# simonrw/rust-tensorflow-serving2

Measured on AMD Instinct MI355X. Metric: Predict RPCs/sec + p50 latency, ResNet-50 batch=1/32 at 1/2/4/8 MI355X, higher is better.
Workload: dtype bf16

## Files before the change

rust_tensorflow_serving2_amd/graph/fused.py:

```python
from __future__ import annotations

import os
from typing import Dict, List, Optional, Sequence, Set, Tuple

import numpy as np
import torch
import torch.nn.functional as F

from ..utils import tensors as T
from . import ops as O
from .ir import Graph, Node
from .placement import to_device, zeros

BF16 = torch.bfloat16
IGEMM_ONLY_ACTS = ("relu6", "hard_swish", "swish")
_CLOSING_ACTS = {"Relu": "relu", "Relu6": "relu6", "_HardSwish": "hard_swish", "_Swish": "swish"}


def _const(g: Graph, ref) -> Optional[torch.Tensor]:
    n = g.nodes.get(ref[0])
    if n is None or n.op != "Const" or n.value is None:
        return None
    v = n.value[ref[1]] if ref[1] < len(n.value) else None
    return v if isinstance(v, torch.Tensor) else None
# ... 78 lines not shown
        del g.nodes[n.name]
    last.op = op
    last.inputs = list(inputs)
    last.ctrl = ctrl
    last.attrs = attrs
    last.value = None
    return last


def _pad_k(w_nk: torch.Tensor, mult: int = 64) -> torch.Tensor:
    n, k = w_nk.shape
    kp = -(-k // mult) * mult
    if kp != k:
        w_nk = torch.cat([w_nk, torch.zeros(n, kp - k, dtype=w_nk.dtype, device=w_nk.device)], dim=1)
    return w_nk


def _to_bf16(x: torch.Tensor) -> torch.Tensor:
    if x.dtype == BF16:
        return x
    if x.dtype == torch.float32 and x.is_cuda and x.is_contiguous():
        from ..ops import hip
        return hip().cast_bf16(x)
    return x.to(BF16).contiguous()


class _Window:

    def _set_window(self, kh: int, kw: int, strides, padding: str, pads):
        self.kh, self.kw = kh, kw
        self.sh, self.sw = strides
        self.padding = padding
        self.pads = pads

    def pads_for(self, h, w):
        if self.padding == "SAME":
            return O.tf_same_pads(h, self.kh, self.sh) + O.tf_same_pads(w, self.kw, self.sw)
        if self.padding == "EXPLICIT":
            return tuple(self.pads)
        return (0, 0, 0, 0)

    def out_hw(self, h, w, pads, kh=None, kw=None):
        pt, pb, pl, pr = pads
        kh, kw = self.kh if kh is None else kh, self.kw if kw is None else kw
        return (h + pt + pb - kh) // self.sh + 1, (w + pl + pr - kw) // self.sw + 1


def _grouped_conv_torch(x: torch.Tensor, w_hwio: torch.Tensor, bias: torch.Tensor, strides, pads, groups: int):
    pt, pb, pl, pr = pads
    xc = x.permute(0, 3, 1, 2)
    xc = F.pad(xc, [pl, pr, pt, pb]) if (pt or pb or pl or pr) else xc
    y = F.conv2d(xc, w_hwio.to(x.dtype).permute(3, 2, 0, 1), stride=tuple(strides), groups=groups)
    return y.permute(0, 2, 3, 1) + bias.to(x.dtype)


class FusedConv(_Window):

    def __init__(self, w_hwio: torch.Tensor, bias: torch.Tensor, strides, padding: str, pads, act: str,
                 device: torch.device, use_hip: bool, name: str):
        kh, kw, self.cin, self.cout = w_hwio.shape
        self._set_window(kh, kw, strides, padding, pads)
        self.act = act
        self.use_hip = use_hip
        self.name = name
        self.device = device
        self.c4 = use_hip and self.cin <= 4 and self.kw <= 8
        self.khp = self.kh + (self.kh % 2) if self.c4 else self.kh
        if use_hip:
            if self.c4:
                w4 = torch.zeros(self.khp, 8, 4, self.cout, device=w_hwio.device)
                w4[:self.kh, :self.kw, :self.cin, :] = w_hwio.float()
                w_nk = w4.permute(3, 0, 1, 2).reshape(self.cout, self.khp * 32)
            else:
                k = self.kh * self.kw * self.cin
                w_nk = w_hwio.permute(3, 0, 1, 2).reshape(self.cout, k)
            self.w = to_device(_pad_k(w_nk).to(BF16), device)
            self.b = to_device(bias.float(), device)
        else:
            self.w_ref = to_device(w_hwio.float(), device)
            self.b_ref = to_device(bias.float(), device)

    post = None
    post_mode = None

    def set_post(self, scale: torch.Tensor, shift: torch.Tensor, act: str, mode: str):
        dev = self.device if self.use_hip else (self.w_ref.device if hasattr(self, "w_ref") else "cpu")
        self.post = (to_device(scale.float(), dev), to_device(shift.float(), dev), act)
        self.post_mode = mode

    def post_ok(self) -> bool:
        return not self.use_hip or (not self.c4 and self.cin % 64 == 0 and self.cout % 8 == 0 and
                                    self.act not in IGEMM_ONLY_ACTS)

    def _hwio(self) -> torch.Tensor:
        if not self.use_hip:
            return self.w_ref
        if self.c4:
            w = self.w[:, :self.khp * 32].reshape(self.cout, self.khp, 8, 4)[:, :self.kh, :self.kw, :self.cin]
        else:
            w = self.w[:, :self.kh * self.kw * self.cin].reshape(self.cout, self.kh, self.kw, self.cin)
        return w.float().permute(1, 2, 3, 0)

    def _torch(self, x, res, pads):
        w = self._hwio().to(x.device)
        b = (self.b if self.use_hip else self.b_ref).to(x.device)
        y = _grouped_conv_torch(x.float(), w, b, (self.sh, self.sw), pads, x.shape[3] // self.cin)
        if res is not None:
            y = y + res.float()
        outs = _with_post(self, _ref_act(y, self.act).contiguous())
        return [o.to(BF16) for o in outs] if self.use_hip else outs

    def __call__(self, ctx, node, ins):
        x = O.to_torch(ins[0])
        res = O.to_torch(ins[1]) if len(ins) > 1 else None
        pt, pb, pl, pr = self.pads_for(x.shape[1], x.shape[2])
        if not self.use_hip or x.shape[3] != self.cin:
            return self._torch(x, res, (pt, pb, pl, pr))
        from ..ops import ACT, hip, tuned_config
        if self.c4:
            ho, wo = self.out_hw(x.shape[1], x.shape[2], (pt, pb, pl, pr))
            hp, wp = (ho - 1) * self.sh + self.khp, (wo - 1) * self.sw + 8
            x = hip().ingest_c4_padded(x.float().contiguous(), hp, wp, pt, pl)
            pt = pb = pl = pr = 0
        elif self.cin % 8 != 0:
            x = x.float().contiguous()
        else:
            x = _to_bf16(x).contiguous()
        H = hip()
        n, h, w, _ = x.shape
        kh, kw = (self.khp, 8) if self.c4 else (self.kh, self.kw)
        ho, wo = self.out_hw(h, w, (pt, pb, pl, pr), kh, kw)
        if res is not None:
            res = _residual_for(res, (n, ho, wo, self.cout))
            if res is None:
                return _add_residual_unfused(self, ctx, node, ins[0], O.to_torch(ins[1]))
            res = _to_bf16(res).contiguous()
        M = n * ho * wo
        args = (x, self.w, self.b, res, kh, kw, self.sh, self.sw, pt, pb, pl, pr, ACT[self.act])
        out = torch.empty((n, ho, wo, self.cout), device=x.device, dtype=BF16)
        K = kh * 32 if self.c4 else kh * kw * self.cin
        dma = not self.c4 and self.cin % 8 == 0
        aligned = (dma and self.cin % 64 == 0) or self.c4
        halo_shape = aligned and not self.c4 and kh == 3 and kw == 3 and self.sh == 1
        halo = halo_shape and self.sw == 1 and pt <= 2 and pl <= 2
        key = ("conv", tuple(x.shape), x.dtype, self.cout, kh, kw, self.sh, res is not None, self.act,
               self.post_mode) + ((self.sw,) if self.sw != self.sh else ()) + \
            (("nohalo",) if halo_shape and self.sw == 1 and not halo else ())
        kw_post, outs = _post_kwargs(self, out)
        run = lambda c, s: H.conv2d(*args, cfg=c, out=out, splits=s, **kw_post)
        flags = {"relu6": True} if self.act in IGEMM_ONLY_ACTS else {}
        cfg, splits = tuned_config(key, M, self.cout, run, K, dma, aligned, halo=halo,
                                   cgemm_only=self.post is not None, stem=self.c4, **flags)
        run(cfg, splits)
        return outs


class FusedDepthwiseConv(_Window):

    MAX_K = 7

    def __init__(self, w_hwc: torch.Tensor, bias: torch.Tensor, strides, padding: str, pads, act: str,
                 device: torch.device, use_hip: bool, name: str):
        kh, kw, self.c = w_hwc.shape
        self._set_window(kh, kw, strides, padding, pads)
        self.act = act
        self.use_hip = use_hip
        self.name = name
        self.device = device
        self.w = to_device(w_hwc.float().contiguous(), device)
        self.b = to_device(bias.float(), device)

    @classmethod
    def hip_ok(cls, kh: int, kw: int, c: int) -> bool:
        return c % 8 == 0 and kh <= cls.MAX_K and kw <= cls.MAX_K

    def _torch(self, x, pads):
        w = self.w.to(x.device).reshape(self.kh, self.kw, 1, self.c)
        return _grouped_conv_torch(x.float(), w, self.b.to(x.device), (self.sh, self.sw), pads, self.c)

    def __call__(self, ctx, node, ins):
        x = O.to_torch(ins[0])
        pt, pb, pl, pr = self.pads_for(x.shape[1], x.shape[2])
        n, h, w, _ = x.shape
        ho, wo = self.out_hw(h, w, (pt, pb, pl, pr))
        if not self.use_hip:
            return [_ref_act(self._torch(x, (pt, pb, pl, pr)), self.act).contiguous()]
        from ..ops import ACT, hip, tuned_choice
        H = hip()
        x = _to_bf16(x).contiguous()
        out = torch.empty((n, ho, wo, self.c), device=x.device, dtype=BF16)

        def run(strip):
            return H.dwconv2d(x, self.w, self.b, self.kh, self.kw, self.sh, self.sw, pt, pl, ho, wo, ACT[self.act],
                              out, strip)
        auto = H.dwconv_strip(n, ho, wo, self.c, self.kh, self.kw, self.sh, self.sw)
        if auto == 0:
            forms = H.dwconv_forms(n, ho, wo, self.c, self.kh, self.kw, self.sh, self.sw)
            if len(forms) == 1:
                return [run(0)]
            key = ("dwconv5x5", tuple(x.shape), self.sh, self.sw, pt, pl, ho, wo, self.act)
            pick = tuned_choice(key, {int(f): (lambda f=int(f): run(f)) for f in forms}, default=0)
            return [run(pick)]
        key = ("dwconv", tuple(x.shape), self.kh, self.kw, self.sh, self.sw, pt, pl, ho, wo, self.act)
# ... 652 lines not shown

    children = ("conv", "pool")

    def __init__(self, conv: FusedConv, pool: MaxPool):
        self.conv, self.pool = conv, pool
        self.use_hip = conv.use_hip and conv.c4

    def accepts_bf16_input(self, pos: int) -> bool:
        return pos == 0 and self.use_hip

    def __call__(self, ctx, node, ins):
        x = O.to_torch(ins[0])
        conv, pool = self.conv, self.pool
        if not (self.use_hip and x.is_cuda and x.dim() == 4):
            return pool(ctx, node, conv(ctx, node, [x]))
        from ..ops import ACT, hip
        pt, pb, pl, pr = conv.pads_for(x.shape[1], x.shape[2])
        hc, wc = conv.out_hw(x.shape[1], x.shape[2], (pt, pb, pl, pr))
        ppt, ppb, ppl, ppr = pool.pads_for(hc, wc)
        kw = {}
        if pool.post is not None:
            sc, sh, act = pool.post
            kw = dict(post_scale=sc, post_shift=sh, post_act=ACT[act])
        x = x.contiguous() if x.dtype == torch.bfloat16 else x.float().contiguous()
        return [hip().stem_pool(x, conv.w, conv.b, pt, pb, pl, pr, ACT[conv.act],
                                ppt, ppb, ppl, ppr, **kw)]


O.OPS["_StemPool"] = _impl_op

CHAIN_SHAPES_ALL = {(64, 256, 64), (64, 256, 128), (128, 512, 128), (128, 512, 256)}
CHAIN_SHAPES_STAGE1 = {(64, 256, 64), (64, 256, 128)}
CHAIN_SHAPES_DUAL = {(128, 256, 64)}
CHAIN_SHAPES_DEFAULT = CHAIN_SHAPES_ALL


class ChainConv:

    children = ("a", "b")

    def __init__(self, a, b: FusedConv):
        self.a, self.b = a, b
        self.dual = isinstance(a, FusedDualConv)
        self.use_hip = a.use_hip and b.use_hip
        self.name = a.name
        if self.dual:
            from types import SimpleNamespace
            self.subs = [(a, SimpleNamespace(op="_FusedDualConv")), (b, SimpleNamespace(op="_FusedConv2D"))]

    def __call__(self, ctx, node, ins):
        x = O.to_torch(ins[0])
        a, b = self.a, self.b

        def split():
            y1 = a(ctx, node, ins)[0]
            return [y1, b(ctx, node, [y1])[0]]
        if self.dual:
            return self._call_dual(x, O.to_torch(ins[1]), split)
        res = O.to_torch(ins[1]) if len(ins) > 1 else None
        if not (self.use_hip and x.is_cuda and x.dim() == 4 and x.shape[-1] == a.cin) or \
                (res is not None and tuple(res.shape) != tuple(x.shape[:3]) + (a.cout,)):
            return split()
        from ..ops import ACT, hip, tuned_choice
        xb = _to_bf16(x).contiguous()
        rb = None if res is None else _to_bf16(res).contiguous()

        def chained():
            return list(hip().conv_chain(xb, a.w, a.b, rb, ACT[a.act], b.w, b.b, ACT[b.act]))
        key = ("chain", tuple(x.shape), a.cout, b.cout, res is not None, a.act, b.act)
        dflt = 1 if (a.cin, a.cout, b.cout) in CHAIN_SHAPES_STAGE1 else 0
        pick = tuned_choice(key, {1: chained, 0: split}, default=dflt)
        return chained() if pick == 1 else split()

    def _call_dual(self, h, x, split):
        a, b = self.a, self.b
        if not (self.use_hip and h.is_cuda and h.dim() == 4 and x.dim() == 4 and h.shape[:3] == x.shape[:3] and
                h.shape[-1] == a.c1 and x.shape[-1] == a.c2):
            return split()
        from ..ops import ACT, hip, tuned_choice
        hb, xb = _to_bf16(h).contiguous(), _to_bf16(x).contiguous()

        def chained():
            return list(hip().conv_chain(hb, a.w, a.b, None, ACT[a.act], b.w, b.b, ACT[b.act], x2=xb))
        key = ("chain", tuple(h.shape), a.cout, b.cout, ("dual", a.c2), a.act, b.act)
        dflt = 1 if (a.c1 + a.c2, a.cout, b.cout) in CHAIN_SHAPES_DUAL else 0
        pick = tuned_choice(key, {1: chained, 0: split}, default=dflt)
        return chained() if pick == 1 else split()


O.OPS["_ChainConv"] = _impl_op
O.OPS["_FusedMatMulLN"] = _impl_op

_PASSTHROUGH = ("Identity", "Squeeze", "Reshape")


def fuse_classifier_head(g, order, fed, fetch_refs, device, opts):
    c = _Ctx(g, order, fed, fetch_refs, device, opts)

    def single(node) -> bool:
        return node.name not in c.fetch_nodes and len(c.cons.get(node.name, [])) == 1

    def walk(ref, chain):
        n = g.nodes.get(ref[0])
        while n is not None and n.op in _PASSTHROUGH and ref[1] == 0 and single(n) and n.inputs:
            chain.append(n)
            ref = n.inputs[0]
            n = g.nodes.get(ref[0])
        return ref, n
# ... 975 lines not shown
```

rust_tensorflow_serving2_amd/kernels/bindings.cpp:

```cpp
#include <cstdlib>
#include <cmath>
#include <algorithm>
#include <torch/extension.h>
#include <ATen/hip/impl/HIPGuardImplMasqueradingAsCUDA.h>
#include <ATen/hip/impl/HIPStreamMasqueradingAsCUDA.h>

#include "common.h"
#include "launch.h"
#include "cgemm.h"

namespace {

using torch::Tensor;

hipStream_t cur_stream(const Tensor& t) {
  return c10::hip::getCurrentHIPStreamMasqueradingAsCUDA(t.device().index()).stream();
}

void check(hipError_t e, const char* what) {
  TORCH_CHECK(e == hipSuccess, what, ": ", hipGetErrorString(e));
}

const tfsk::TileConfig* config_of(int64_t cfg) {
  return cfg >= 0 && cfg < tfsk::kTileIdEnd ? tfsk::tile_config(int(cfg)) : nullptr;
// ... 611 lines not shown
  check(tfsk::stem_pool_launch(xin.data_ptr(), xb16, bf16p(w), int(w.size(1)), bias.data_ptr<float>(), bf16p_mut(y), N,
                               H, W, C, cout, int(PT), int(PL), Hc, Wc, int(PPT), int(PPL), Hp, Wp, int(act), sc, sh,
                               int(post_act), cur_stream(x)), "stem_pool");
  return y;
}

std::vector<Tensor> conv_chain(const Tensor& x, const Tensor& w1, const Tensor& b1,
                               const c10::optional<Tensor>& residual, int64_t act1, const Tensor& w2,
                               const Tensor& b2, int64_t act2, const c10::optional<Tensor>& x2) {
  need(x, at::kBFloat16, "x");
  need(w1, at::kBFloat16, "w1");
  need(w2, at::kBFloat16, "w2");
  need(b1, at::kFloat, "b1");
  need(b2, at::kFloat, "b2");
  TORCH_CHECK(x.dim() == 4, "conv_chain: x must be NHWC");
  const bool dual = x2.has_value();
  const int Ka = x.size(3);
  const uint16_t* x2p = nullptr;
  if (dual) {
    need(*x2, at::kBFloat16, "x2");
    TORCH_CHECK(x2->dim() == 4 && x2->size(0) == x.size(0) && x2->size(1) == x.size(1) && x2->size(2) == x.size(2),
                "conv_chain: x2 must have x's n, h, w");
    TORCH_CHECK(Ka % 64 == 0 && x2->size(3) % 64 == 0 && x2->size(3) > 0,
                "conv_chain: both sources' channels must be multiples of 64");
    TORCH_CHECK(x2->device() == x.device(), "conv_chain: tensors on different devices");
    x2p = bf16p(*x2);
  }
  const int K1 = Ka + (dual ? int(x2->size(3)) : 0), N1 = w1.size(0), N2 = w2.size(0);
  TORCH_CHECK(w1.dim() == 2 && w2.dim() == 2 && w1.size(1) >= K1 && w2.size(1) >= N1 && w1.size(1) % 8 == 0 &&
                  w2.size(1) % 8 == 0, "conv_chain: w1 [N1][>= K1], w2 [N2][>= N1]");
  TORCH_CHECK(tfsk::conv_chain_supported(K1, N1, N2, dual), "conv_chain: unsupported shape K1=", K1, " N1=", N1,
              " N2=", N2, dual ? " (dual)" : "");
  TORCH_CHECK(b1.numel() == N1 && b2.numel() == N2, "conv_chain: bias sizes");
  TORCH_CHECK(w1.device() == x.device() && w2.device() == x.device() && b1.device() == x.device() &&
                  b2.device() == x.device(), "conv_chain: tensors on different devices");
  const uint16_t* rp = nullptr;
  if (residual.has_value()) {
    need(*residual, at::kBFloat16, "residual");
    TORCH_CHECK(residual->dim() == 4 && residual->size(0) == x.size(0) && residual->size(1) == x.size(1) &&
                    residual->size(2) == x.size(2) && residual->size(3) == N1, "conv_chain: residual [n][h][w][N1]");
    rp = bf16p(*residual);
  }
  c10::hip::HIPGuardMasqueradingAsCUDA guard(x.device());
  const int M = x.size(0) * x.size(1) * x.size(2);
  Tensor y1 = torch::empty({x.size(0), x.size(1), x.size(2), N1}, x.options());
  Tensor y2 = torch::empty({x.size(0), x.size(1), x.size(2), N2}, x.options());
  check(tfsk::conv_chain_launch(bf16p(x), bf16p(w1), int(w1.size(1)), b1.data_ptr<float>(), rp, bf16p_mut(y1),
                                bf16p(w2), int(w2.size(1)), b2.data_ptr<float>(), bf16p_mut(y2), M, K1, N1, N2,
                                int(act1), int(act2), cur_stream(x), x2p, Ka),
        "conv_chain");
  return {y1, y2};
}

Tensor global_avgpool(const Tensor& x, const c10::optional<Tensor>& out) {
  need(x, at::kBFloat16, "x");
  TORCH_CHECK(x.dim() == 4 && x.size(3) % 8 == 0, "global_avgpool: NHWC with C % 8 == 0");
  c10::hip::HIPGuardMasqueradingAsCUDA guard(x.device());
  const int N = x.size(0), HW = x.size(1) * x.size(2), C = x.size(3);
  Tensor y = out.has_value() ? *out : torch::empty({N, C}, x.options());
  need(y, at::kBFloat16, "out");
  check(tfsk::global_avgpool_nhwc_launch(bf16p(x), bf16p_mut(y), N, HW, C, cur_stream(x)), "gap");
  return y;
}

std::vector<Tensor> softmax_argmax(const Tensor& logits, bool want_probs, bool want_classes,
                                   const c10::optional<Tensor>& probs_out,
                                   const c10::optional<Tensor>& classes_out) {
  TORCH_CHECK(logits.is_cuda() && logits.dim() >= 1 && logits.stride(-1) == 1 &&
                  (logits.is_contiguous() || logits.dim() == 2),
              "logits must be a GPU tensor with unit column stride (contiguous, or 2-D with a row stride)");
  const bool bf = logits.scalar_type() == at::kBFloat16;
  TORCH_CHECK(bf || logits.scalar_type() == at::kFloat, "logits must be f32 or bf16");
  c10::hip::HIPGuardMasqueradingAsCUDA guard(logits.device());
  const int cols = logits.size(-1);
  const int rows = logits.numel() / cols;
  const long ld = logits.dim() == 2 ? long(logits.stride(0)) : long(cols);
  TORCH_CHECK(ld >= cols, "logits row stride");
  Tensor probs, classes;
  if (want_probs) {
    probs = probs_out.has_value() ? *probs_out : torch::empty(logits.sizes(), logits.options().dtype(at::kFloat));
    need(probs, at::kFloat, "probs");
  }
  if (want_classes) {
    auto sz = logits.sizes().vec();
    sz.pop_back();
    classes = classes_out.has_value() ? *classes_out : torch::empty(sz, logits.options().dtype(at::kLong));
    need(classes, at::kLong, "classes");
  }
  check(tfsk::softmax_argmax_launch(logits.data_ptr(), bf, want_probs ? probs.data_ptr<float>() : nullptr,
                                    want_classes ? classes.data_ptr<int64_t>() : nullptr, rows, cols, ld,
                                    cur_stream(logits)), "softmax_argmax");
  return {probs, classes};
}

std::tuple<Tensor, Tensor, bool> classifier_head_impl(const Tensor& x, const Tensor& w, const Tensor& bias, int64_t n,
                                                      int64_t probs_host, int64_t classes_host);

std::vector<Tensor> classifier_head(const Tensor& x, const Tensor& w, const Tensor& bias, int64_t n) {
  auto r = classifier_head_impl(x, w, bias, n, 0, 0);
  return {std::get<0>(r), std::get<1>(r)};
}

std::tuple<Tensor, Tensor, bool> classifier_head_impl(const Tensor& x, const Tensor& w, const Tensor& bias, int64_t n,
                                                      int64_t probs_host, int64_t classes_host) {
  need(x, at::kBFloat16, "x");
  need(w, at::kBFloat16, "w");
// ... 278 lines not shown
              "window_attention: operands must be smaller than 2 GiB");
  TORCH_CHECK(aligned16(qkv), "window_attention: qkv must be 16-byte aligned");
  TORCH_CHECK(aligned16(bias), "window_attention: bias must be 16-byte aligned");
  Tensor y = out.has_value() ? *out : torch::empty({R, heads * D}, qkv.options());
  need(y, at::kBFloat16, "out");
  TORCH_CHECK(y.numel() == R * heads * D, "window_attention: out has the wrong size");
  TORCH_CHECK(aligned16(y), "window_attention: out must be 16-byte aligned");
  TORCH_CHECK(tfsk::window_attention_supported(R, S, heads, D, nW, g.Hf, g.Wf, g.ws, g.shift),
              "window_attention: unsupported launch");
  check(tfsk::window_attention_launch(bf16p(qkv), bias.data_ptr<float>(), mp, bf16p_mut(y), R, int(S), int(heads),
                                      int(nW), float(scale), int(g.Hf), int(g.Wf), int(g.ws), int(g.shift),
                                      cur_stream(qkv)),
        "window_attention");
  return y;
}

Tensor patch_tokens(const Tensor& x, const Tensor& table, const c10::optional<Tensor>& out) {
  need(x, at::kBFloat16, "x");
  need(table, at::kFloat, "table");
  TORCH_CHECK(x.dim() == 3, "patch_tokens: x must be [B, P, C]");
  TORCH_CHECK(table.dim() == 2 && table.size(0) == x.size(1) + 1 && table.size(1) == x.size(2),
              "patch_tokens: table must be [P + 1, C]");
  const int64_t B = x.size(0), P = x.size(1), C = x.size(2);
  TORCH_CHECK(C % 8 == 0, "patch_tokens: C % 8 != 0 (C = ", C, ")");
  TORCH_CHECK(aligned16(x), "patch_tokens: x must be 16-byte aligned");
  TORCH_CHECK(aligned16(table), "patch_tokens: table must be 16-byte aligned");
  c10::hip::HIPGuardMasqueradingAsCUDA guard(x.device());
  Tensor y = out.has_value() ? *out : torch::empty({B, P + 1, C}, x.options());
  need(y, at::kBFloat16, "out");
  TORCH_CHECK(y.numel() == B * (P + 1) * C, "patch_tokens: out has the wrong size");
  TORCH_CHECK(aligned16(y), "patch_tokens: out must be 16-byte aligned");
  TORCH_CHECK(tfsk::patch_tokens_supported(B, P, C), "patch_tokens: operands must be smaller than 2 GiB");
  check(tfsk::patch_tokens_launch(bf16p(x), table.data_ptr<float>(), bf16p_mut(y), B, P, C, cur_stream(x)),
        "patch_tokens");
  return y;
}

}

PYBIND11_MODULE(TORCH_EXTENSION_NAME, m) {
  m.doc() = "gfx950 HIP kernels (MFMA implicit-GEMM conv/GEMM, attention, norms, pooling)";
  m.def("conv2d", &conv2d, "NHWC implicit-GEMM conv (+bias +residual +act)", py::arg("x"), py::arg("w"),
        py::arg("bias"), py::arg("residual"), py::arg("kh"), py::arg("kw"), py::arg("sh"), py::arg("sw"),
        py::arg("pt"), py::arg("pb"), py::arg("pl"), py::arg("pr"), py::arg("act") = 0, py::arg("cfg") = 0,
        py::arg("out") = py::none(), py::arg("out_f32") = false, py::arg("splits") = 1,
        py::arg("post_scale") = py::none(), py::arg("post_shift") = py::none(), py::arg("post_act") = 0,
        py::arg("out2") = py::none(), py::arg("post_only") = false);
  m.def("conv_chain", &conv_chain, "expand 1x1 (+residual, act) -> next reduce 1x1 (+act) in one kernel",
        py::arg("x"), py::arg("w1"), py::arg("b1"), py::arg("residual"), py::arg("act1"), py::arg("w2"),
        py::arg("b2"), py::arg("act2"), py::arg("x2") = py::none());
  m.def("conv_chain_supported", [](int64_t k1, int64_t n1, int64_t n2, bool dual) {
    return tfsk::conv_chain_supported(int(k1), int(n1), int(n2), dual);
  }, py::arg("k1"), py::arg("n1"), py::arg("n2"), py::arg("dual") = false);
  m.def("conv2d_dual", &conv2d_dual, "act(conv1x1(h) + conv1x1_stride(x) + bias) as one K-concatenated GEMM",
        py::arg("h"), py::arg("x"), py::arg("w"), py::arg("bias"), py::arg("sh"), py::arg("sw"), py::arg("act") = 0,
        py::arg("cfg") = 36, py::arg("out") = py::none(), py::arg("splits") = 1,
        py::arg("post_scale") = py::none(), py::arg("post_shift") = py::none(), py::arg("post_act") = 0,
        py::arg("out2") = py::none(), py::arg("post_only") = false);
  m.def("linear_lnx", &linear_lnx,
        "GEMM whose A / residual rows are LayerNorm inputs (statistics as partials), optionally "
        "returning its own rows' partials: {y, partials}",
        py::arg("x"), py::arg("w"), py::arg("bias"), py::arg("residual"), py::arg("act"), py::arg("cfg"),
        py::arg("out_f32") = false, py::arg("out") = py::none(), py::arg("a_st") = py::none(),
        py::arg("a_colsum") = py::none(), py::arg("a_eps") = 1e-12, py::arg("r_st") = py::none(),
        py::arg("r_gamma") = py::none(), py::arg("r_beta") = py::none(), py::arg("r_eps") = 1e-12,
        py::arg("stats") = false);
  m.def("linear", &linear,"x @ w^T (+bias +residual +act)", py::arg("x"), py::arg("w"), py::arg("bias"),
        py::arg("residual") = py::none(), py::arg("act") = 0, py::arg("cfg") = 0, py::arg("out_f32") = false,
        py::arg("alpha") = 1.0, py::arg("out") = py::none(), py::arg("splits") = 1);
  m.def("stem_pool", &stem_pool, py::arg("x"), py::arg("w"), py::arg("bias"), py::arg("pt"), py::arg("pb"),
        py::arg("pl"), py::arg("pr"), py::arg("act"), py::arg("ppt"), py::arg("ppb"), py::arg("ppl"), py::arg("ppr"),
        py::arg("post_scale") = py::none(), py::arg("post_shift") = py::none(), py::arg("post_act") = 0);
  m.def("maxpool", &maxpool, py::arg("x"), py::arg("kh"), py::arg("kw"), py::arg("sh"), py::arg("sw"),
        py::arg("pt"), py::arg("pb"), py::arg("pl"), py::arg("pr"), py::arg("out") = py::none(),
        py::arg("post_scale") = py::none(), py::arg("post_shift") = py::none(), py::arg("post_act") = 0);
  m.def("dwconv2d", &dwconv2d, "depthwise conv: act(conv(x, w [KH*KW][C] f32) + bias), NHWC bf16", py::arg("x"),
        py::arg("w"), py::arg("bias"), py::arg("kh"), py::arg("kw"), py::arg("sh"), py::arg("sw"), py::arg("pt"),
        py::arg("pl"), py::arg("ho"), py::arg("wo"), py::arg("act") = 0, py::arg("out") = py::none(),
        py::arg("strip") = 0);
  m.def("dwconv_strip", [](int64_t n, int64_t ho, int64_t wo, int64_t c, int64_t kh, int64_t kw, int64_t sh,
                           int64_t sw) {
    return tfsk::dwconv_strip(int(n), int(ho), int(wo), int(c), int(kh), int(kw), int(sh), int(sw));
  }, "output rows per thread dwconv2d picks by itself (0: the generic kernel, which has no strips)");
  m.def("dwconv_forms", [](int64_t n, int64_t ho, int64_t wo, int64_t c, int64_t kh, int64_t kw, int64_t sh,
                           int64_t sw) {
    int forms[tfsk::kDwMaxForms];
    const int k = tfsk::dwconv_forms(int(n), int(ho), int(wo), int(c), int(kh), int(kw), int(sh), int(sw), forms);
    return std::vector<int64_t>(forms, forms + k);
  }, "the strip values dwconv2d takes for the shape: [0], [0, 2, 8] (3 x 3 strips) or [0, 2, 4] (5 x 5 strips)");
  m.def("dwconv_ln", &dwconv_ln, "depthwise 7x7 conv + bias + LayerNorm over C in one launch, NHWC bf16",
        py::arg("x"), py::arg("w"), py::arg("bias"), py::arg("gamma"), py::arg("beta"), py::arg("eps"), py::arg("pt"),
        py::arg("pl"), py::arg("ho"), py::arg("wo"), py::arg("out") = py::none(), py::arg("kh") = 7,
        py::arg("kw") = 7, py::arg("sh") = 1, py::arg("sw") = 1);
  m.def("dwconv_ln_supported", [](int64_t n, int64_t ho, int64_t wo, int64_t c, int64_t kh, int64_t kw, int64_t sh,
                                  int64_t sw) {
    return tfsk::dwconv_ln_supported(n, ho, wo, c, int(kh), int(kw), int(sh), int(sw));
  }, "whether dwconv_ln takes the shape: 7 x 7, stride 1, C % 8 == 0, 8 <= C <= dwconv_ln_max_c");
  m.def("dwconv_ln_grid", [](int64_t n, int64_t ho, int64_t wo, int64_t c) {
    return int64_t(tfsk::dwconv_ln_grid(n, ho, wo, c));
  }, "workgroups of the dwconv_ln launch for the shape (0: nothing to launch or unsupported)");
  m.attr("dwconv_ln_max_c") = int64_t(tfsk::kDwLnMaxC);
  m.def("gconv2d", &gconv2d, "grouped 3x3 conv on MFMA: act(conv(x, w packed bf16) + bias), NHWC bf16", py::arg("x"),
        py::arg("w"), py::arg("bias"), py::arg("cg"), py::arg("sh"), py::arg("pt"), py::arg("pl"), py::arg("ho"),
        py::arg("wo"), py::arg("act") = 0, py::arg("out") = py::none(), py::arg("cg_out") = -1, py::arg("sw") = -1,
        py::arg("kh") = 3, py::arg("kw") = 3);
  m.def("gconv_supported", [](int64_t c, int64_t cg_in, int64_t cg_out, int64_t kh, int64_t kw, int64_t sh,
// ... 138 lines not shown
```

rust_tensorflow_serving2_amd/kernels/launch.h:

```cpp
#pragma once
#include <hip/hip_runtime.h>
#include <stdint.h>

#include "tile_configs.h"

namespace tfsk {

struct IGemmArgs {
  const void* a;
  const uint16_t* b;
  int M, N, K;
  int lda, ldb;
  int H, W, C, KH, KW, SH, SW, PT, PL, Ho, Wo;
  const float* bias;
  const uint16_t* residual;
  int ldr;
  int act;
  void* out;
  int ldc;
  int out_f32;
  float alpha;
  int splits;
  int kt_per_split;
  float* ws;
// ... 2 lines not shown
  const void* a2;
  int64_t a2_bytes;
  int K1;
  int TH, TW, TI;
  void* out2;
  const float* scale2;
  const float* shift2;
  int act2;
  int* counters;
  long long* trace;
  int trace_cap;
  int epi_f32;
  float* st_out;
  const float* a_st;
  const float* a_colsum;
  int a_parts;
  float a_eps;
  const float* r_st;
  const float* r_gamma;
  const float* r_beta;
  int r_parts;
  float r_eps;
};

int* splitk_counters(int n, hipStream_t s);
void splitk_counters_prepare(hipStream_t s);
void splitk_counters_set_owner(int64_t owner);
void splitk_counters_add_stream(int64_t owner, hipStream_t s);
int64_t splitk_counters_release(int64_t owner);
int64_t splitk_counters_reclaim();
int64_t splitk_counters_pending();
int64_t splitk_counters_captured_in_use();

enum AMode : int { kADense = 0, kAIm2col = 1, kAStemF32 = 2, kAStem7x7x3 = 3, kAC4 = 4, kADual = 5 };

hipError_t ingest_c4_launch(const float* x, uint16_t* y, int64_t pixels, int C, hipStream_t stream);

hipError_t ingest_c4_pad_launch(const float* x, uint16_t* y, int N, int H, int W, int C, int Hp, int Wp, int pt,
                               int pl, hipStream_t stream);

hipError_t splitk_reduce_launch(const IGemmArgs& args, hipStream_t stream);

hipError_t igemm_launch(const IGemmArgs& args, int a_mode, int cfg, hipStream_t stream);

hipError_t stem_pool_launch(const void* x, bool x_bf16, const uint16_t* w, int ldw, const float* bias, uint16_t* y,
                            int N, int H, int W, int C, int cout, int pt, int pl, int Hc, int Wc, int ppt, int ppl,
                            int Hp, int Wp, int act, const float* pscale, const float* pshift, int pact,
                            hipStream_t s);
bool conv_chain_supported(int K1, int N1, int N2, bool dual = false);
hipError_t conv_chain_launch(const uint16_t* x, const uint16_t* w1, int ldw1, const float* b1, const uint16_t* res,
                             uint16_t* y1, const uint16_t* w2, int ldw2, const float* b2, uint16_t* y2, int M, int K1,
                             int N1, int N2, int act1, int act2, hipStream_t s, const uint16_t* x2 = nullptr,
                             int K1a = 0);
hipError_t maxpool_nhwc_launch(const uint16_t* x, uint16_t* y, int N, int H, int W, int C,
                               int KH, int KW, int SH, int SW, int PT, int PL, int Ho, int Wo,
                               hipStream_t stream, const float* scale = nullptr, const float* shift = nullptr,
                               int act = 0);
constexpr int kDwStripShort = 2, kDwStripTall = 8;
constexpr int kDwStrip5Short = 2, kDwStrip5Tall = 4;
constexpr int kDwMaxForms = 3;
int dwconv_strip(int N, int Ho, int Wo, int C, int KH, int KW, int SH, int SW, int strip = 0);
int dwconv_forms(int N, int Ho, int Wo, int C, int KH, int KW, int SH, int SW, int* forms);
hipError_t dwconv_nhwc_launch(const uint16_t* x, const float* w, const float* bias, uint16_t* y, int N, int H, int W,
                              int C, int KH, int KW, int SH, int SW, int PT, int PL, int Ho, int Wo, int act,
                              int strip, hipStream_t stream);
constexpr int kDwLnMaxC = 1024;
constexpr int kDwLnRowsTall = 4, kDwLnRowsShort = 2;
bool dwconv_ln_supported(long N, long Ho, long Wo, long C, int KH, int KW, int SH, int SW);
long dwconv_ln_grid(long N, long Ho, long Wo, long C);
hipError_t dwconv_ln_launch(const uint16_t* x, const float* w, const float* bias, const float* gamma,
                            const float* beta, uint16_t* y, int N, int H, int W, int C, int KH, int KW, int SH, int SW,
                            int PT, int PL, int Ho, int Wo, float eps, hipStream_t stream);
constexpr int kGconvSlab = 32;
constexpr int gconv_ksteps(int cg) { return (9 * cg + 31) / 32; }
bool gconv_supported(int C, int CGin, int CGout, int KH, int KW, int SH, int SW);
long gconv_packed_elems(int C, int CG);
hipError_t gconv_nhwc_launch(const uint16_t* x, const uint16_t* w, const float* bias, uint16_t* y, int N, int H, int W,
                             int C, int CGin, int CGout, int KH, int KW, int SH, int SW, int PT, int PL, int Ho,
                             int Wo, int act, hipStream_t stream);
constexpr int kSeMaxC = 2048, kSeMaxCr = 512;
bool se_gate_supported(long B, long HW, long C, long Cr);
hipError_t se_gate_launch(const uint16_t* x, const float* w1, const float* b1, const float* w2, const float* b2,
                          float* gate, int B, int HW, int C, int Cr, int act1, int gate_act, hipStream_t stream);
hipError_t se_scale_launch(const uint16_t* x, const float* gate, uint16_t* y, int B, int HW, int C,
                           hipStream_t stream);
hipError_t global_avgpool_nhwc_launch(const uint16_t* x, uint16_t* y, int N, int HW, int C,
                                      hipStream_t stream);
hipError_t classifier_head_launch(const uint16_t* x, const uint16_t* w, const float* bias, float* ws,
                                  float* probs, int64_t* classes, int M, int HW, int K, int Np, int N,
                                  hipStream_t s, int* counter = nullptr, float* probs_h = nullptr,
                                  int64_t* classes_h = nullptr);
size_t classifier_head_ws_floats(int M, int K, int Np);
bool classifier_head_one_launch(int M, int HW, int K, int Np, int N);
hipError_t dense_softmax_launch(const float* x, int ldx, const uint16_t* w, int ldw, const float* bias,
                                float* probs, int rows, int N, int K, hipStream_t s);
hipError_t key_mask_adder_launch(const void* m, int is_int, float one, float scale, float* out, int64_t n,
                                 hipStream_t s);
hipError_t softmax_argmax_launch(const void* logits, int in_bf16, float* probs, int64_t* classes,
                                 int rows, int cols, long ld, hipStream_t stream);
hipError_t cast_f32_bf16_launch(const float* x, uint16_t* y, int64_t n, hipStream_t stream);
hipError_t cast_bf16_f32_launch(const uint16_t* x, float* y, int64_t n, hipStream_t stream);
int epi_f32_env();
hipError_t h2d_rows_launch(const void* host, void* dev, int64_t bytes, hipStream_t stream);

hipError_t layernorm_launch(const uint16_t* x, const uint16_t* r, const float* gamma, const float* beta,
                            uint16_t* y, int rows, int cols, float eps, hipStream_t stream);
// ... 46 lines not shown
```

Measured before the change: 57100.

## Add row-panel 1x1 conv kernel keeping A in registers for wide expansions

```diff
diff --git a/rust_tensorflow_serving2_amd/graph/fused.py b/rust_tensorflow_serving2_amd/graph/fused.py
--- a/rust_tensorflow_serving2_amd/graph/fused.py
+++ b/rust_tensorflow_serving2_amd/graph/fused.py
@@ -154,6 +154,18 @@
     xc = F.pad(xc, [pl, pr, pt, pb]) if (pt or pb or pl or pr) else xc
     y = F.conv2d(xc, w_hwio.to(x.dtype).permute(3, 2, 0, 1), stride=tuple(strides), groups=groups)
     return y.permute(0, 2, 3, 1) + bias.to(x.dtype)
+
+
+_PANEL = os.environ.get("TFSERVE_PANEL", "1") != "0"
+
+
+def panel_eligible(kh, kw, sh, sw, pads, cin, cout, act, post=None, c4=False) -> bool:
+    return (kh == 1 and kw == 1 and sh == 1 and sw == 1 and not any(pads) and cin in (128, 256, 512) and
+            cout % 64 == 0 and cout >= 2 * cin and act in ("none", "relu") and post is None and not c4)
+
+
+def panel_key(x_shape, cout, has_res, act):
+    return ("panel", tuple(x_shape), cout, bool(has_res), act)
 
 
 class FusedConv(_Window):
@@ -212,12 +224,32 @@
         outs = _with_post(self, _ref_act(y, self.act).contiguous())
         return [o.to(BF16) for o in outs] if self.use_hip else outs
 
-    def __call__(self, ctx, node, ins):
+    def panel_choice(self, ctx, node, ins) -> Optional[int]:
+        x = O.to_torch(ins[0])
+        res = O.to_torch(ins[1]) if len(ins) > 1 else None
+        if not (_PANEL and self.use_hip and x.is_cuda and x.dim() == 4 and x.shape[3] == self.cin):
+            return None
+        if not panel_eligible(self.kh, self.kw, self.sh, self.sw, self.pads_for(x.shape[1], x.shape[2]), self.cin,
+                              self.cout, self.act, self.post, self.c4):
+            return None
+        if res is not None and tuple(res.shape) != tuple(x.shape[:3]) + (self.cout,):
+            return None
+        from ..ops import hip, tuned_choice
+        forms = hip().conv1x1_panel_forms(x.shape[0] * x.shape[1] * x.shape[2], self.cout, self.cin)
+        if not forms:
+            return None
+        opts = {i: (lambda i=i: self(ctx, node, ins, panel_pick=i)) for i in range(len(forms) + 1)}
+        pick = tuned_choice(panel_key(x.shape, self.cout, res is not None, self.act), opts, default=0)
+        return pick if pick in opts else 0
+
+    def __call__(self, ctx, node, ins, panel_pick=None):
         x = O.to_torch(ins[0])
         res = O.to_torch(ins[1]) if len(ins) > 1 else None
         pt, pb, pl, pr = self.pads_for(x.shape[1], x.shape[2])
         if not self.use_hip or x.shape[3] != self.cin:
             return self._torch(x, res, (pt, pb, pl, pr))
+        if panel_pick is None:
+            panel_pick = self.panel_choice(ctx, node, ins)
         from ..ops import ACT, hip, tuned_config
         if self.c4:
             ho, wo = self.out_hw(x.shape[1], x.shape[2], (pt, pb, pl, pr))
@@ -251,6 +283,10 @@
         kw_post, outs = _post_kwargs(self, out)
         run = lambda c, s: H.conv2d(*args, cfg=c, out=out, splits=s, **kw_post)
         flags = {"relu6": True} if self.act in IGEMM_ONLY_ACTS else {}
+        if panel_pick:
+            bm, ns = H.conv1x1_panel_forms(M, self.cout, self.cin)[panel_pick - 1]
+            H.conv1x1_panel(x, self.w, self.b, res, ACT[self.act], bm, ns, out=out)
+            return outs
         cfg, splits = tuned_config(key, M, self.cout, run, K, dma, aligned, halo=halo,
                                    cgemm_only=self.post is not None, stem=self.c4, **flags)
         run(cfg, splits)
@@ -1009,8 +1045,10 @@
         x = O.to_torch(ins[0])
         a, b = self.a, self.b
 
+        pp = a.panel_choice(ctx, node, ins) if isinstance(a, FusedConv) else None
+
         def split():
-            y1 = a(ctx, node, ins)[0]
+            y1 = (a(ctx, node, ins) if pp is None else a(ctx, node, ins, panel_pick=pp))[0]
             return [y1, b(ctx, node, [y1])[0]]
         if self.dual:
             return self._call_dual(x, O.to_torch(ins[1]), split)
diff --git a/rust_tensorflow_serving2_amd/kernels/bindings.cpp b/rust_tensorflow_serving2_amd/kernels/bindings.cpp
--- a/rust_tensorflow_serving2_amd/kernels/bindings.cpp
+++ b/rust_tensorflow_serving2_amd/kernels/bindings.cpp
@@ -687,6 +687,40 @@
   return {y1, y2};
 }
 
+Tensor conv1x1_panel(const Tensor& x, const Tensor& w, const Tensor& bias, const c10::optional<Tensor>& residual,
+                     int64_t act, int64_t bm, int64_t nsplit, const c10::optional<Tensor>& out) {
+  need(x, at::kBFloat16, "x");
+  need(w, at::kBFloat16, "w");
+  need(bias, at::kFloat, "bias");
+  TORCH_CHECK(x.dim() == 4, "conv1x1_panel: x must be NHWC");
+  const int64_t M64 = x.size(0) * x.size(1) * x.size(2);
+  const int K = x.size(3), N = w.size(0);
+  TORCH_CHECK(w.dim() == 2 && w.size(1) >= K && w.size(1) % 8 == 0, "conv1x1_panel: w [N][>= K, a multiple of 8]");
+  TORCH_CHECK(M64 < (int64_t(1) << 31) && tfsk::conv1x1_panel_supported(int(M64), N, K, int(bm), int(nsplit)),
+              "conv1x1_panel: unsupported shape M=", M64, " N=", N, " K=", K, " bm=", bm, " nsplit=", nsplit);
+  TORCH_CHECK(act == tfsk::kActNone || act == tfsk::kActRelu, "conv1x1_panel: act must be none or relu");
+  TORCH_CHECK(bias.numel() == N, "conv1x1_panel: bias size");
+  TORCH_CHECK(w.device() == x.device() && bias.device() == x.device(), "conv1x1_panel: tensors on different devices");
+  const uint16_t* rp = nullptr;
+  if (residual.has_value()) {
+    need(*residual, at::kBFloat16, "residual");
+    TORCH_CHECK(residual->dim() == 4 && residual->size(0) == x.size(0) && residual->size(1) == x.size(1) &&
+                    residual->size(2) == x.size(2) && residual->size(3) == N && residual->device() == x.device(),
+                "conv1x1_panel: residual [n][h][w][N]");
+    rp = bf16p(*residual);
+  }
+  c10::hip::HIPGuardMasqueradingAsCUDA guard(x.device());
+  Tensor y = out.has_value() ? *out : torch::empty({x.size(0), x.size(1), x.size(2), N}, x.options());
+  need(y, at::kBFloat16, "out");
+  TORCH_CHECK(y.numel() == M64 * N && y.device() == x.device(), "conv1x1_panel: out [n][h][w][N]");
+  TORCH_CHECK(aligned16(x) && aligned16(w) && aligned16(bias) && aligned16(y) && (!rp || aligned16(*residual)),
+              "conv1x1_panel: operands must be 16-byte aligned");
+  check(tfsk::conv1x1_panel_launch(bf16p(x), bf16p(w), int(w.size(1)), bias.data_ptr<float>(), rp, bf16p_mut(y),
+                                   int(M64), N, K, int(bm), int(nsplit), int(act), cur_stream(x)),
+        "conv1x1_panel");
+  return y;
+}
+
 Tensor global_avgpool(const Tensor& x, const c10::optional<Tensor>& out) {
   need(x, at::kBFloat16, "x");
   TORCH_CHECK(x.dim() == 4 && x.size(3) % 8 == 0, "global_avgpool: NHWC with C % 8 == 0");
@@ -1071,6 +1105,24 @@
   m.def("conv_chain_supported", [](int64_t k1, int64_t n1, int64_t n2, bool dual) {
     return tfsk::conv_chain_supported(int(k1), int(n1), int(n2), dual);
   }, py::arg("k1"), py::arg("n1"), py::arg("n2"), py::arg("dual") = false);
+  m.def("conv1x1_panel", &conv1x1_panel, "wide 1x1 conv (+residual, act) on the row-panel kernel: A read once",
+        py::arg("x"), py::arg("w"), py::arg("bias"), py::arg("residual"), py::arg("act"), py::arg("bm"),
+        py::arg("nsplit"), py::arg("out") = py::none());
+  m.def("conv1x1_panel_supported", [](int64_t m, int64_t n, int64_t k, int64_t bm, int64_t nsplit, int64_t act,
+                                      const c10::optional<int64_t>& res_stride) {
+    return m < (int64_t(1) << 31) && n < (int64_t(1) << 31) &&
+           tfsk::conv1x1_panel_supported(int(m), int(n), int(k), int(bm), int(nsplit)) &&
+           (act == tfsk::kActNone || act == tfsk::kActRelu) && (!res_stride.has_value() || *res_stride == n);
+  }, py::arg("m"), py::arg("n"), py::arg("k"), py::arg("bm"), py::arg("nsplit"), py::arg("act") = 0,
+        py::arg("res_stride") = py::none());
+  m.def("conv1x1_panel_forms", [](int64_t m, int64_t n, int64_t k) {
+    int bm[tfsk::kPanelMaxForms], ns[tfsk::kPanelMaxForms];
+    std::vector<std::pair<int64_t, int64_t>> forms;
+    if (m >= (int64_t(1) << 31) || n >= (int64_t(1) << 31)) return forms;
+    const int c = tfsk::conv1x1_panel_forms(int(m), int(n), int(k), bm, ns);
+    for (int i = 0; i < c; ++i) forms.emplace_back(bm[i], ns[i]);
+    return forms;
+  }, "the (bm, nsplit) forms of conv1x1_panel worth timing for an M x N x K conv (none: unsupported)");
   m.def("conv2d_dual", &conv2d_dual, "act(conv1x1(h) + conv1x1_stride(x) + bias) as one K-concatenated GEMM",
         py::arg("h"), py::arg("x"), py::arg("w"), py::arg("bias"), py::arg("sh"), py::arg("sw"), py::arg("act") = 0,
         py::arg("cfg") = 36, py::arg("out") = py::none(), py::arg("splits") = 1,
diff --git a/rust_tensorflow_serving2_amd/kernels/launch.h b/rust_tensorflow_serving2_amd/kernels/launch.h
--- a/rust_tensorflow_serving2_amd/kernels/launch.h
+++ b/rust_tensorflow_serving2_amd/kernels/launch.h
@@ -78,6 +78,11 @@
                              uint16_t* y1, const uint16_t* w2, int ldw2, const float* b2, uint16_t* y2, int M, int K1,
                              int N1, int N2, int act1, int act2, hipStream_t s, const uint16_t* x2 = nullptr,
                              int K1a = 0);
+constexpr int kPanelMaxForms = 6;
+bool conv1x1_panel_supported(int M, int N, int K, int bm, int nsplit);
+int conv1x1_panel_forms(int M, int N, int K, int* bm, int* nsplit);
+hipError_t conv1x1_panel_launch(const uint16_t* a, const uint16_t* w, int ldw, const float* bias, const uint16_t* res,
+                                uint16_t* out, int M, int N, int K, int bm, int nsplit, int act, hipStream_t s);
 hipError_t maxpool_nhwc_launch(const uint16_t* x, uint16_t* y, int N, int H, int W, int C,
                                int KH, int KW, int SH, int SW, int PT, int PL, int Ho, int Wo,
                                hipStream_t stream, const float* scale = nullptr, const float* shift = nullptr,
diff --git a/rust_tensorflow_serving2_amd/kernels/panel.hip b/rust_tensorflow_serving2_amd/kernels/panel.hip
--- /dev/null
+++ b/rust_tensorflow_serving2_amd/kernels/panel.hip
@@ -0,0 +1,262 @@
+#include <type_traits>
+#include <utility>
+
+#include "gemm_common.h"
+
+namespace tfsk {
+namespace {
+
+using namespace gemm;
+
+template <class F, int... I>
+__device__ __forceinline__ void static_for(F&& f, std::integer_sequence<int, I...>) {
+  (f(std::integral_constant<int, I>{}), ...);
+}
+
+__device__ __forceinline__ void slab_read8(const float* src, f32x4& lo, f32x4& hi) {
+  typedef __attribute__((address_space(3))) const float* lds_cfp_t;
+  const uint32_t addr = uint32_t(reinterpret_cast<uintptr_t>((lds_cfp_t)src));
+  asm volatile("ds_read_b128 %0, %2\n\tds_read_b128 %1, %2 offset:16\n\ts_waitcnt lgkmcnt(0)"
+               : "=&v"(lo), "=&v"(hi)
+               : "v"(addr)
+               : "memory");
+}
+
+struct PanelArgs {
+  const uint16_t* a;
+  const uint16_t* w;
+  const float* bias;
+  const uint16_t* res;
+  uint16_t* out;
+  int M, N, ldw;
+  int ns_log2;
+  float lo;
+};
+
+constexpr int kPanelNT = 256, kPanelStgLd = 68;
+
+template <int K, int BM>
+struct PN {
+  static constexpr int KT1 = K / KT;
+  static constexpr int KS = K / 32;
+  static constexpr int RPW = BM / 4, TM = RPW / 16;
+  static constexpr int S = 4;
+  static constexpr int SLOT = 64 * KT * 2;
+  static constexpr int WPW = 64 / 8 / 4;
+  static constexpr int RING = S * SLOT;
+  static constexpr int STG = 4 * 16 * kPanelStgLd * 4;
+  static constexpr int LDS = RING + STG;
+  static constexpr int EPI = 2 * TM + 2;
+  static constexpr int STORES = 2 * TM;
+  static constexpr int younger(int u) {
+    int pf = 0;
+    for (int d = 1; d <= S - 2; ++d) pf += ((u - d) % KT1 + KT1) % KT1 == 0;
+    return (S - 2) * WPW + pf * EPI;
+  }
+  static_assert(K % KT == 0 && (KT1 & (KT1 - 1)) == 0 && (BM == 64 || BM == 128), "panel shape");
+  static_assert((S & (S - 1)) == 0, "slot = t & (S - 1)");
+  static_assert(LDS <= 80 * 1024, "two workgroups per CU");
+  static_assert((S - 2) * WPW + (S - 2) * EPI < 64, "vmcnt range");
+};
+
+template <int K, int BM>
+__global__ __launch_bounds__(kPanelNT, 2) void conv1x1_panel_kernel(PanelArgs p) {
+  using G = PN<K, BM>;
+  extern __shared__ __attribute__((aligned(16))) char smem[];
+  typedef __attribute__((address_space(3))) void* lds_ptr_t;
+  const int tid = threadIdx.x, lane = tid & 63;
+  const int wid = __builtin_amdgcn_readfirstlane(tid >> 6);
+  const int fr = lane & 15, fq = lane >> 4;
+  const int prow = lane >> 3;
+  const uint32_t kc = uint32_t(((lane & 7) ^ prow) * 8);
+  const int c8 = lane & 7, rl = lane >> 3;
+  const int M = p.M, N = p.N;
+
+  const int id = xcd_remap(blockIdx.x, gridDim.x);
+  const int panel = id >> p.ns_log2, span = id - (panel << p.ns_log2);
+  const int m0 = panel * BM;
+  const int NS = N >> p.ns_log2;
+  const int n0 = span * NS;
+  const int ntiles = NS >> 6;
+  const int T = ntiles * G::KT1;
+
+  const __amdgpu_buffer_rsrc_t rsA =
+      __builtin_amdgcn_make_buffer_rsrc(const_cast<uint16_t*>(p.a), 0, int(long(M) * K * 2), 0x00020000);
+  const __amdgpu_buffer_rsrc_t rsW =
+      __builtin_amdgcn_make_buffer_rsrc(const_cast<uint16_t*>(p.w), 0, int(long(N) * p.ldw * 2), 0x00020000);
+  const __amdgpu_buffer_rsrc_t rsB =
+      __builtin_amdgcn_make_buffer_rsrc(const_cast<float*>(p.bias), 0, N * 4, 0x00020000);
+  const __amdgpu_buffer_rsrc_t rsR = __builtin_amdgcn_make_buffer_rsrc(
+      const_cast<uint16_t*>(p.res), 0, p.res ? int(long(M) * N * 2) : 0, 0x00020000);
+  const __amdgpu_buffer_rsrc_t rsO = __builtin_amdgcn_make_buffer_rsrc(p.out, 0, int(long(M) * N * 2), 0x00020000);
+
+  bf16x8 af[G::TM][G::KS];
+#pragma unroll
+  for (int i = 0; i < G::TM; ++i) {
+    const int m = m0 + wid * G::RPW + i * 16 + fr;
+#pragma unroll
+    for (int ks = 0; ks < G::KS; ++ks) {
+      const uint32_t v = m < M ? (uint32_t(m) * uint32_t(K) + uint32_t(ks * 32 + fq * 8)) * 2u : kOOB;
+      af[i][ks] = __builtin_bit_cast(bf16x8, __builtin_amdgcn_raw_buffer_load_b128(rsA, v, 0, 0));
+    }
+  }
+
+  auto issue_w = [&](int t) {
+    const int j = t / G::KT1, kt = t % G::KT1;
+    char* slot = smem + (t & (G::S - 1)) * G::SLOT;
+    const uint32_t past = t < T ? 0u : kOOB;
+#pragma unroll
+    for (int q = 0; q < G::WPW; ++q) {
+      const int pc = wid * G::WPW + q;
+      const int n = n0 + j * 64 + pc * 8 + prow;
+      const uint32_t v = ((uint32_t(n) * uint32_t(p.ldw) + uint32_t(kt * KT) + kc) * 2u) | past;
+      __builtin_amdgcn_raw_ptr_buffer_load_lds(rsW, (lds_ptr_t)(slot + pc * 1024), 16, v, 0, 0, 0);
+    }
+  };
+
+  auto load_epi = [&](int j, u32x4 (&rr)[G::TM][2], u32x4 (&bb)[2]) {
+    const uint32_t past = j < ntiles ? 0u : kOOB;
+    const uint32_t n = uint32_t(n0 + j * 64 + c8 * 8);
+    bb[0] = __builtin_amdgcn_raw_buffer_load_b128(rsB, (n * 4u) | past, 0, 0);
+    bb[1] = __builtin_amdgcn_raw_buffer_load_b128(rsB, (n * 4u + 16u) | past, 0, 0);
+#pragma unroll
+    for (int i = 0; i < G::TM; ++i)
+#pragma unroll
+      for (int k = 0; k < 2; ++k) {
+        const int m = m0 + wid * G::RPW + i * 16 + rl + 8 * k;
+        rr[i][k] = __builtin_amdgcn_raw_buffer_load_b128(
+            rsR, (m < M ? (uint32_t(m) * uint32_t(N) + n) * 2u : kOOB) | past, 0, 0);
+      }
+  };
+
+  float* stg = reinterpret_cast<float*>(smem + G::RING) + wid * 16 * kPanelStgLd;
+  const uint32_t ro0 = uint32_t((fr * KT + ((fq ^ (fr & 7)) * 8)) * 2);
+  const uint32_t ro1 = uint32_t((fr * KT + (((4 + fq) ^ (fr & 7)) * 8)) * 2);
+  const float lo_act = p.lo;
+
+  auto tile = [&](int j, u32x4 (&rc)[G::TM][2], u32x4 (&bc)[2], u32x4 (&rn)[G::TM][2], u32x4 (&bn)[2]) {
+    f32x4 acc[G::TM][4];
+#pragma unroll
+    for (int i = 0; i < G::TM; ++i)
+#pragma unroll
+      for (int jj = 0; jj < 4; ++jj) acc[i][jj] = f32x4{0.f, 0.f, 0.f, 0.f};
+    static_for([&](auto uc) __attribute__((always_inline)) {
+      constexpr int u = decltype(uc)::value;
+      const int t = j * G::KT1 + u;
+      wait_vmcnt<G::younger(u)>();
+      lds_barrier();
+      issue_w(t + G::S - 1);
+      if (u == 0) load_epi(j + 1, rn, bn);
+      const char* sb = smem + (t & (G::S - 1)) * G::SLOT;
+#pragma unroll
+      for (int kk = 0; kk < 2; ++kk) {
+        bf16x8 bfr[4];
+#pragma unroll
+        for (int jj = 0; jj < 4; ++jj)
+          bfr[jj] = *reinterpret_cast<const bf16x8*>(sb + (kk ? ro1 : ro0) + jj * 16 * KT * 2);
+#pragma unroll
+        for (int i = 0; i < G::TM; ++i)
+#pragma unroll
+          for (int jj = 0; jj < 4; ++jj)
+            acc[i][jj] = __builtin_amdgcn_mfma_f32_16x16x32_bf16(af[i][u * 2 + kk], bfr[jj], acc[i][jj], 0, 0, 0);
+      }
+    }, std::make_integer_sequence<int, G::KT1>{});
+    const float bv[8] = {__uint_as_float(bc[0].x), __uint_as_float(bc[0].y), __uint_as_float(bc[0].z),
+                         __uint_as_float(bc[0].w), __uint_as_float(bc[1].x), __uint_as_float(bc[1].y),
+                         __uint_as_float(bc[1].z), __uint_as_float(bc[1].w)};
+    const uint32_t n = uint32_t(n0 + j * 64 + c8 * 8);
+#pragma unroll
+    for (int i = 0; i < G::TM; ++i) {
+#pragma unroll
+      for (int jj = 0; jj < 4; ++jj)
+#pragma unroll
+        for (int r = 0; r < 4; ++r) stg[(fq * 4 + r) * kPanelStgLd + jj * 16 + fr] = acc[i][jj][r];
+      __builtin_amdgcn_wave_barrier();
+#pragma unroll
+      for (int k = 0; k < 2; ++k) {
+        const float* src = stg + (rl + 8 * k) * kPanelStgLd + c8 * 8;
+        f32x4 lo, hi;
+        slab_read8(src, lo, hi);
+        const float a[8] = {lo.x, lo.y, lo.z, lo.w, hi.x, hi.y, hi.z, hi.w};
+        const u32x4 w = rc[i][k];
+        const uint32_t rw[4] = {w.x, w.y, w.z, w.w};
+        u32x4 ov;
+#pragma unroll
+        for (int e = 0; e < 4; ++e) {
+          const float v0 = fmaxf(a[2 * e] + bv[2 * e] + __uint_as_float(rw[e] << 16), lo_act);
+          const float v1 = fmaxf(a[2 * e + 1] + bv[2 * e + 1] + __uint_as_float(rw[e] & 0xffff0000u), lo_act);
+          ov[e] = pack_bf16x2(v0, v1);
+        }
+        const int m = m0 + wid * G::RPW + i * 16 + rl + 8 * k;
+        __builtin_amdgcn_raw_buffer_store_b128(ov, rsO, m < M ? (uint32_t(m) * uint32_t(N) + n) * 2u : kOOB, 0, 0);
+      }
+      __builtin_amdgcn_wave_barrier();
+    }
+  };
+
+#pragma unroll
+  for (int s = 0; s < G::S - 1; ++s) issue_w(s);
+  u32x4 r0[G::TM][2], b0[2], r1[G::TM][2], b1[2];
+  load_epi(0, r0, b0);
+  wait_vmcnt<0>();
+  __syncthreads();
+
+  int j = 0;
+  for (; j + 1 < ntiles; j += 2) {
+    tile(j, r0, b0, r1, b1);
+    tile(j + 1, r1, b1, r0, b0);
+  }
+  if (j < ntiles) tile(j, r0, b0, r1, b1);
+  wait_vmcnt<0>();
+}
+
+template <int K, int BM>
+hipError_t launch_panel(const PanelArgs& a, int nsplit, hipStream_t s) {
+  using G = PN<K, BM>;
+  hipError_t e = ensure_dyn_lds(reinterpret_cast<const void*>(&conv1x1_panel_kernel<K, BM>), G::LDS);
+  if (e != hipSuccess) return e;
+  const int grid = ((a.M + BM - 1) / BM) * nsplit;
+  hipLaunchKernelGGL((conv1x1_panel_kernel<K, BM>), dim3(grid), dim3(kPanelNT), G::LDS, s, a);
+  return hipGetLastError();
+}
+
+}
+
+bool conv1x1_panel_supported(int M, int N, int K, int bm, int nsplit) {
+  if (M <= 0 || (K != 128 && K != 256 && K != 512) || N <= 0 || N % 64) return false;
+  if (nsplit != 1 && nsplit != 2 && nsplit != 4 && nsplit != 8) return false;
+  if (N % nsplit || (N / nsplit) % 64) return false;
+  if (bm != 64 && !(bm == 128 && K <= 256)) return false;
+  return long(M) * N * 2 < 0x7fffffffL && long(M) * K * 2 < 0x7fffffffL;
+}
+
+int conv1x1_panel_forms(int M, int N, int K, int* bm, int* nsplit) {
+  int count = 0;
+  for (int pass = 0; pass < 2 && count == 0; ++pass)
+    for (int ns = 1; ns <= 8; ns *= 2)
+      for (int b = 64; b <= 128; b += 64) {
+        if (!conv1x1_panel_supported(M, N, K, b, ns)) continue;
+        const long wgs = long((M + b - 1) / b) * ns;
+        if ((pass == 0 && wgs < 128) || count == kPanelMaxForms) continue;
+        bm[count] = b;
+        nsplit[count] = ns;
+        ++count;
+      }
+  return count;
+}
+
+hipError_t conv1x1_panel_launch(const uint16_t* a, const uint16_t* w, int ldw, const float* bias, const uint16_t* res,
+                                uint16_t* out, int M, int N, int K, int bm, int nsplit, int act, hipStream_t s) {
+  if (M == 0) return hipSuccess;
+  if (!conv1x1_panel_supported(M, N, K, bm, nsplit) || ldw < K || ldw % 8) return hipErrorInvalidValue;
+  if (act != kActNone && act != kActRelu) return hipErrorInvalidValue;
+  if (long(N + 256) * ldw * 2 >= 0x7fffffffL) return hipErrorInvalidValue;
+  const int ns_log2 = nsplit == 1 ? 0 : nsplit == 2 ? 1 : nsplit == 4 ? 2 : 3;
+  const PanelArgs p{a, w, bias, res, out, M, N, ldw, ns_log2, act == kActRelu ? 0.f : -INFINITY};
+  if (bm == 128) return K == 128 ? launch_panel<128, 128>(p, nsplit, s) : launch_panel<256, 128>(p, nsplit, s);
+  if (K == 128) return launch_panel<128, 64>(p, nsplit, s);
+  if (K == 256) return launch_panel<256, 64>(p, nsplit, s);
+  return launch_panel<512, 64>(p, nsplit, s);
+}
+
+}
```

After: 58710 (median of 6 runs). 1.03x the previous value.
